# 0xC000005/PyChebyshev

Measured on AMD Instinct MI355X. Metric: point-evals/sec, 5D Black-Scholes n=11^5 barycentric + TT, 1/2/4/8 GPU, higher is better.
Workload: dtype f64; 1 GPU; 5D Black-Scholes n=11^5 full-tensor barycentric, 1,000,000 fp64 queries per GPU; evals_per_point=1, parallelism=batch-sharded x1, model replicated, one process per GPU, gather=none

## Files before the change

include/pcx.h:

```cpp
#ifndef PCX_H
#define PCX_H

#include <stddef.h>
#include <stdint.h>

#ifdef __cplusplus
extern "C" {
#endif

#define PCX_ABI_VERSION 1

#define PCX_OK 0
#define PCX_ERR_INVALID (-1)
#define PCX_ERR_NO_DEVICE (-2)
#define PCX_ERR_HIP (-3)
#define PCX_ERR_UNSUPPORTED (-4)
#define PCX_ERR_NOMEM (-5)

#define PCX_MAX_DIMS 16

typedef struct pcx_bary pcx_bary;
typedef struct pcx_tt pcx_tt;
typedef struct pcx_spline pcx_spline;
typedef struct pcx_slider pcx_slider;
// ... 47 lines not shown
int pcx_bary_derivative_tensor(pcx_bary *h, const int32_t *deriv, double *tensor_out);

int pcx_bary_chebyshev_coefficients(pcx_bary *h, double *coeffs_out);

int pcx_bary_sobol(pcx_bary *h, double *variance_out, double *first_out, double *total_out);

int pcx_tensor_contract_axis(int device, int d, const int32_t *n_nodes, const double *tensor,
                             int axis, const double *vec, double *out);

int pcx_bary_set_kernel(pcx_bary *h, int variant);
int pcx_bary_count_gemms(pcx_bary *h, const int32_t *derivs, int m, int64_t N, int32_t *gemms_out);
int pcx_bary_set_group_tolerance(pcx_bary *h, double tol);
int pcx_bary_set_group_span(pcx_bary *h, int span);
int pcx_bary_kernel_info(pcx_bary *h, int32_t *info_out );
int pcx_bary_grid_info(pcx_bary *h, int32_t *info_out );
int pcx_bary_stream(pcx_bary *h, void **stream);

int pcx_spline_create(int device, int d, const int32_t *n_knots, const double *knots_cat,
                      pcx_bary *const *pieces, int n_pieces, pcx_spline **out);
int pcx_spline_destroy(pcx_spline *h);
int pcx_spline_eval_batch(pcx_spline *h, const double *pts, int64_t N, const int32_t *deriv,
                          double *out);
int pcx_spline_eval_multi_batch(pcx_spline *h, const double *pts, int64_t N, const int32_t *derivs,
                                int m, double *out);
int pcx_spline_piece_ids(pcx_spline *h, const double *pts, int64_t N, int32_t *ids_out);
int pcx_spline_eval_batch_dev(pcx_spline *h, const double *d_pts, int64_t N, const int32_t *deriv,
                              double *d_out);
int pcx_spline_eval_multi_batch_dev(pcx_spline *h, const double *d_pts, int64_t N,
                                    const int32_t *derivs, int m, double *d_out);

// ... 87 lines not shown
```

pychebyshev_amd/_lib.py:

```python
from __future__ import annotations

import ctypes
import os

import numpy as np

HERE = os.path.dirname(os.path.abspath(__file__))
LIB_PATH = os.path.join(HERE, "libpcx_hip.so")

PCX_OK = 0
PCX_ERR_INVALID = -1
PCX_ERR_NO_DEVICE = -2
PCX_ERR_HIP = -3
PCX_ERR_UNSUPPORTED = -4
PCX_ERR_NOMEM = -5


class PcxLibraryError(RuntimeError):
    """libpcx_hip.so is missing, stale, or there is no usable MI355X device."""


class PcxError(RuntimeError):

    def __init__(self, code: int, message: str):
# ... 46 lines not shown
    "pcx_bary_eval_multi_batch_dev": (_I, [_V, _V, _L, c_i32p, _I, _V, _V]),
    "pcx_bary_group_eval_multi_batch": (_I, [c_vpp, _I, c_f64p, _L, c_i32p, _I, c_f64p, _I]),
    "pcx_bary_derivative_tensor": (_I, [_V, c_i32p, c_f64p]),
    "pcx_bary_chebyshev_coefficients": (_I, [_V, c_f64p]),
    "pcx_bary_sobol": (_I, [_V, c_f64p, c_f64p, c_f64p]),
    "pcx_cheb1d_calculus": (_I, [_I, _I, _D, _D, c_f64p, c_f64p, c_f64p, c_f64p, _L, _I, c_f64p, c_i32p, c_f64p, c_f64p]),
    "pcx_bary_calculus_batch": (_I, [_V, _I, c_f64p, c_f64p, c_f64p, _L, _I, c_f64p, c_i32p, c_f64p, c_f64p]),
    "pcx_tt_calculus_batch": (_I, [_V, _I, c_f64p, _L, _I, c_f64p, c_i32p, c_f64p, c_f64p]),
    "pcx_tensor_contract_axis": (_I, [_I, _I, c_i32p, c_f64p, _I, c_f64p, c_f64p]),
    "pcx_bary_set_kernel": (_I, [_V, _I]),
    "pcx_bary_set_group_span": (_I, [_V, _I]),
    "pcx_bary_count_gemms": (_I, [_V, c_i32p, _I, _L, c_i32p]),
    "pcx_bary_set_group_tolerance": (_I, [_V, _D]),
    "pcx_bary_kernel_info": (_I, [_V, c_i32p]),
    "pcx_bary_grid_info": (_I, [_V, c_i32p]),
    "pcx_bary_stream": (_I, [_V, c_vpp]),
    "pcx_spline_create": (_I, [_I, _I, c_i32p, c_f64p, c_vpp, _I, c_vpp]),
    "pcx_spline_destroy": (_I, [_V]),
    "pcx_spline_eval_batch": (_I, [_V, c_f64p, _L, c_i32p, c_f64p]),
    "pcx_spline_eval_multi_batch": (_I, [_V, c_f64p, _L, c_i32p, _I, c_f64p]),
    "pcx_spline_piece_ids": (_I, [_V, c_f64p, _L, c_i32p]),
    "pcx_spline_eval_batch_dev": (_I, [_V, _V, _L, c_i32p, _V]),
    "pcx_spline_eval_multi_batch_dev": (_I, [_V, _V, _L, c_i32p, _I, _V]),
    "pcx_slider_create": (_I, [_I, _I, _I, c_vpp, c_i32p, c_i32p, _D, c_vpp]),
    "pcx_slider_destroy": (_I, [_V]),
    "pcx_slider_eval_batch": (_I, [_V, c_f64p, _L, c_i32p, c_f64p]),
    "pcx_slider_eval_multi_batch": (_I, [_V, c_f64p, _L, c_i32p, _I, c_f64p]),
    "pcx_slider_eval_multi_batch_dev": (_I, [_V, _V, _L, c_i32p, _I, _V]),
    "pcx_tt_create": (_I, [_I, _I, c_i32p, c_i32p, c_f64p, c_f64p, c_f64p, c_i32p, c_vpp]),
    "pcx_tt_destroy": (_I, [_V]),
# ... 139 lines not shown
```

pychebyshev_amd/csrc/bary_kernels.h:

```cpp
#pragma once

#include "pcx_common.h"

static __global__ void k_mode_product(const double *__restrict__ in, double *__restrict__ out,
                               const double *__restrict__ D, long outer, int na, long inner) {
    long idx = (long)blockIdx.x * blockDim.x + threadIdx.x;
    long total = outer * na * inner;
    if (idx >= total) return;
    long q = idx % inner;
    long t = idx / inner;
    int i = (int)(t % na);
    long o = t / na;
    const double *src = in + (o * na) * inner + q;
    const double *drow = D + (long)i * na;
    double s = 0.0;
    for (int j = 0; j < na; ++j) s = __builtin_fma(src[(long)j * inner], drow[j], s);
    out[idx] = s;
}

static __global__ void k_contract_axis(const double *__restrict__ in, double *__restrict__ out,
                                const double *__restrict__ vec, long outer, int na, long inner) {
    long idx = (long)blockIdx.x * blockDim.x + threadIdx.x;
    if (idx >= outer * inner) return;
    long q = idx % inner;
// ... 104 lines not shown
    const uint4 q = reinterpret_cast<const uint4 *>(codes)[4 * t + g];
    return pcx_u4{{q.x, q.y, q.z, q.w}};
}

typedef const pcx_d4 __attribute__((address_space(1))) *pcx_seed_ptr;
template <int R>
struct pcx_seed { pcx_d4 v[R > 0 ? R : 1]; };
template <int R>
__device__ __forceinline__ pcx_seed<R> load_seed(pcx_seed_ptr seed, long t, int g) {
    pcx_seed<R> q;
#pragma unroll
    for (int r = 0; r < R; ++r) q.v[r] = seed[(4 * t + g) * R + r];
    return q;
}

template <int NF>
__device__ __forceinline__ double code_weight_t(unsigned code, const double *bw_col, int PW) {
    if constexpr (NF >= 4) return code_weight(code, bw_col, PW);
    else {
        double w0 = bw_col[(code & 255u) * PW];
        double w1 = bw_col[((code >> 8) & 255u) * PW];
        if constexpr (NF == 3) return (w0 * w1) * bw_col[((code >> 16) & 255u) * PW];
        else return w0 * w1;
    }
}

#define PCX_CHUNK_TILES 4

template <int KS, int NT, bool WIDE, int NF = 4, bool G0 = false, int R = 0>
__global__ void __launch_bounds__(256, 2)
k_bary_mfma(BaryDims dims, BaryMfmaPlan plan, const double *__restrict__ nodes,
            const double *__restrict__ wts, const double *const *__restrict__ frag_tab,
            const unsigned *__restrict__ rowcode, const unsigned *__restrict__ kcode,
            const unsigned *__restrict__ rowcode_hi, const unsigned *__restrict__ kcode_hi,
            const double *__restrict__ pts, double *__restrict__ out, long N, long ostride,
            long ooff, int chunks_per_split, double *__restrict__ partial,
            const int *__restrict__ perm, BaryG0 gs, const double *__restrict__ diff0) {
    static_assert(NT == 1 || NT == 2 || NT == 4, "PW must divide the wave");
    constexpr int PW = 16 * NT;
    constexpr int PH = 64 / PW;
    extern __shared__ double lds[];
    const int lane = threadIdx.x & 63;
    const int wave = threadIdx.x >> 6;
    const int g = lane >> 4;
    const int c = lane & 15;
    double *bw = lds + (size_t)wave * plan.rows * PW;
    const double *bwt = bw + (size_t)plan.tail_base * PW;
    const long base = ((long)blockIdx.x * 4 + wave) * PW;
    typedef const double __attribute__((address_space(1))) *gptr_t;
    const gptr_t frag = (gptr_t)frag_tab[blockIdx.z];
    const pcx_seed_ptr seed = (pcx_seed_ptr)(frag + (size_t)plan.MT * KS * 64);
    const int nchunks = (plan.MT + PCX_CHUNK_TILES - 1) / PCX_CHUNK_TILES;
    const int ch0 = blockIdx.y * chunks_per_split;
    const int ch1 = (ch0 + chunks_per_split < nchunks) ? ch0 + chunks_per_split : nchunks;

    {
        const int pp = lane % PW;
        const int ph = lane / PW;
        const long pidx = base + pp;
        const bool valid = pidx < N;
        const long row = valid ? (perm ? (long)perm[pidx] : pidx) : 0;
        for (int k = ph; k < dims.d; k += PH) {
            const double *nd = nodes + dims.off[k];
            double x = valid ? pts[row * dims.d + k] : nd[0];
            const int trow = dims.off[k] + (k >= plan.split ? 1 : 0);
            bary_weights_1d(x, nd, wts + dims.off[k], dims.n[k], bw + (size_t)trow * PW + pp, PW);
        }
        if (ph == 0) {
            bw[(size_t)(plan.tail_base - 1) * PW + pp] = 1.0;
            bw[(size_t)(plan.rows - 1) * PW + pp] = 1.0;
        }
    }
    __syncthreads();

    double B[NT][KS];
#pragma unroll
    for (int s = 0; s < KS; ++s) {
        unsigned code = kcode[4 * s + g];
#pragma unroll
        for (int nt = 0; nt < NT; ++nt) B[nt][s] = code_weight(code, bwt + 16 * nt + c, PW);
        if (WIDE) {
            unsigned hi = kcode_hi[4 * s + g];
#pragma unroll
            for (int nt = 0; nt < NT; ++nt) B[nt][s] *= code_weight(hi, bwt + 16 * nt + c, PW);
        }
    }
    double ws[NT][R > 0 ? R : 1];
#pragma unroll
    for (int r = 0; r < R; ++r) {
        unsigned code = kcode[4 * KS + r];
#pragma unroll
        for (int nt = 0; nt < NT; ++nt) ws[nt][r] = code_weight(code, bwt + 16 * nt + c, PW);
        if (WIDE) {
            unsigned hi = kcode_hi[4 * KS + r];
#pragma unroll
            for (int nt = 0; nt < NT; ++nt) ws[nt][r] *= code_weight(hi, bwt + 16 * nt + c, PW);
        }
    }

    double total[NT], cs[NT];
#pragma unroll
    for (int nt = 0; nt < NT; ++nt) { total[nt] = 0.0; cs[nt] = 0.0; }
    const gptr_t tf = frag + lane;
    const int t_begin = ch0 * PCX_CHUNK_TILES;
    const int t_end = (ch1 * PCX_CHUNK_TILES < plan.MT) ? ch1 * PCX_CHUNK_TILES : plan.MT;
    const bool split = gridDim.y > 1;
    constexpr bool PIPELINED = (KS >= 12);
    constexpr int DEPTH = 6;
    unsigned cn[4] = {0u, 0u, 0u, 0u}, cnh[4] = {0u, 0u, 0u, 0u};
    double head[DEPTH];
    pcx_d4 acc[NT];
    auto seed_acc = [&](const pcx_seed<R> &sd) {
#pragma unroll
        for (int nt = 0; nt < NT; ++nt) acc[nt] = (pcx_d4){0.0, 0.0, 0.0, 0.0};
#pragma unroll
        for (int r = 0; r < R; ++r)
#pragma unroll
            for (int nt = 0; nt < NT; ++nt)
#pragma unroll
                for (int j = 0; j < 4; ++j) acc[nt][j] = __builtin_fma(sd.v[r][j], ws[nt][r], acc[nt][j]);
    };
    constexpr bool CARRY = PIPELINED && R > 0;
#pragma unroll
    for (int i = 0; i < DEPTH; ++i) head[i] = 0.0;
    if (PIPELINED && t_begin < t_end) {
        if constexpr (R > 0) seed_acc(load_seed<R>(seed, t_begin, g));
        {
            const pcx_u4 q = load_row_codes(rowcode, t_begin, g);
            pcx_u4 qh = q;
            if (WIDE) qh = load_row_codes(rowcode_hi, t_begin, g);
#pragma unroll
            for (int j = 0; j < 4; ++j) {
                cn[j] = q.v[j];
                if (WIDE) cnh[j] = qh.v[j];
            }
        }
#pragma unroll
        for (int i = 0; i < DEPTH; ++i) head[i] = tf[((size_t)t_begin * KS + i) * 64];
    }
    for (int t = t_begin; t < t_end; ++t) {
        double w[NT][4];
        pcx_seed<R> sdn;
        if constexpr (!CARRY) {
            if constexpr (R > 0) sdn = load_seed<R>(seed, t, g);
            seed_acc(sdn);
        }
        const gptr_t tt = tf + (size_t)t * KS * 64;
        if constexpr (PIPELINED) {
            const int t_next = (t + 1 < t_end) ? t + 1 : t;
            const gptr_t tn = tf + (size_t)t_next * KS * 64;
            double ring[DEPTH];
            unsigned cc[4], cch[4];
#pragma unroll
            for (int i = 0; i < DEPTH; ++i) ring[i] = head[i];
            {
                const pcx_u4 q = load_row_codes(rowcode, t_next, g);
                pcx_u4 qh = q;
                if (WIDE) qh = load_row_codes(rowcode_hi, t_next, g);
#pragma unroll
                for (int j = 0; j < 4; ++j) {
                    cc[j] = cn[j];
                    cn[j] = q.v[j];
                    if (WIDE) { cch[j] = cnh[j]; cnh[j] = qh.v[j]; }
                }
            }
            double wr[4][NT][4];
            double wh[4][NT][4];
#pragma unroll
            for (int s = 0; s < KS; ++s) {
                const double a = ring[s % DEPTH];
                if (s + DEPTH < KS) ring[s % DEPTH] = tt[(s + DEPTH) * 64];
                else head[s + DEPTH - KS] = tn[(s + DEPTH - KS) * 64];
                if constexpr (R > 0) {
                    if (s == KS - DEPTH) sdn = load_seed<R>(seed, t_next, g);
                }
#pragma unroll
                for (int j = 0; j < 4; ++j) {
                    if (s == 2 * j) {
#pragma unroll
                        for (int nt = 0; nt < NT; ++nt)
#pragma unroll
                            for (int f = 0; f < (NF < 4 ? NF : 4); ++f)
                                wr[j][nt][f] = bw[(size_t)((cc[j] >> (8 * f)) & 255u) * PW + 16 * nt + c];
                    }
                    if (s == 2 * j + 2) {
#pragma unroll
                        for (int nt = 0; nt < NT; ++nt)
                            w[nt][j] = NF >= 4 ? (wr[j][nt][0] * wr[j][nt][1]) * (wr[j][nt][2] * wr[j][nt][3])
                                     : (NF == 3 ? (wr[j][nt][0] * wr[j][nt][1]) * wr[j][nt][2]
                                                : wr[j][nt][0] * wr[j][nt][1]);
                    }
                    if (WIDE && s == 2 * j + 1) {
#pragma unroll
                        for (int nt = 0; nt < NT; ++nt)
#pragma unroll
                            for (int f = 0; f < 4; ++f)
                                wh[j][nt][f] = bw[(size_t)((cch[j] >> (8 * f)) & 255u) * PW + 16 * nt + c];
                    }
// ... 48 lines not shown
                    v += __shfl_xor(v, 32, 64);
                    if (g == 0) Pl[(size_t)i0 * PW + 16 * nt + c] = v;
                    cs[nt] = 0.0;
                }
            }
            continue;
        }
        const bool chunk_end = ((t + 1) % PCX_CHUNK_TILES == 0) || (t + 1 == plan.MT);
        if (chunk_end) {
            if (split) {
                const int ch = t / PCX_CHUNK_TILES;
#pragma unroll
                for (int nt = 0; nt < NT; ++nt) {
                    long pidx = base + 16 * nt + c;
                    if (pidx < N)
                        partial[(((size_t)blockIdx.z * nchunks + ch) * 4 + g) * (size_t)N + pidx] = cs[nt];
                }
            }
#pragma unroll
            for (int nt = 0; nt < NT; ++nt) { total[nt] += cs[nt]; cs[nt] = 0.0; }
        }
    }

    if constexpr (G0) {
        if (lane < PW) {
            double *Pl = const_cast<double *>(bwt) + lane;
            const long pidx = base + lane;
            const long row = (pidx < N) ? (perm ? (long)perm[pidx] : pidx) : 0;
            bary_g0_finish(gs, diff0, Pl, Pl + (size_t)gs.n0 * PW, bw + (size_t)dims.off[0] * PW + lane, PW,
                           pidx < N ? out + row * ostride + ooff : nullptr);
        }
// ... 161 lines not shown
    }

#pragma unroll
    for (int nt = 0; nt < NT; ++nt) {
        double v = total[nt];
        v += __shfl_xor(v, 16, 64);
        v += __shfl_xor(v, 32, 64);
        long pidx = base + 16 * nt + c;
        if (g == 0 && pidx < N) {
            long row = perm ? (long)perm[pidx] : pidx;
            out[row * ostride + ooff + blockIdx.z] = v;
        }
    }
}

static __global__ void k_bary_reduce(const double *__restrict__ partial, double *__restrict__ out, long N,
                              int nchunks, int nspec, long ostride, long ooff,
                              const int *__restrict__ perm) {
    long idx = (long)blockIdx.x * blockDim.x + threadIdx.x;
    if (idx >= N * nspec) return;
    long p = idx % N;
    int z = (int)(idx / N);
    const double *src = partial + (size_t)z * nchunks * 4 * (size_t)N + p;
    double sg[4];
    for (int g = 0; g < 4; ++g) {
        double t = 0.0;
        for (int ch = 0; ch < nchunks; ++ch) t += src[((size_t)ch * 4 + g) * (size_t)N];
        sg[g] = t;
    }
    long row = perm ? (long)perm[p] : p;
    out[row * ostride + ooff + z] = (sg[0] + sg[1]) + (sg[2] + sg[3]);
}

static __global__ void __launch_bounds__(256)
k_bary_rows(BaryDims dims, int LPP, const double *__restrict__ nodes,
            const double *__restrict__ wts, const double *__restrict__ T,
            const double *__restrict__ pts, double *__restrict__ out, long N, long ostride,
            long ooff, const int *__restrict__ perm) {
    extern __shared__ double lds[];
    const int ppw = 256 / LPP;
    const int pl = threadIdx.x / LPP;
    const int sub = threadIdx.x % LPP;
    const long pidx = (long)blockIdx.x * ppw + pl;
    const bool valid = pidx < N;
    const long row = valid ? (perm ? (long)perm[pidx] : pidx) : 0;
    double *bw = lds + (size_t)pl * dims.sum_n;
// ... 298 lines not shown
```

pychebyshev_amd/csrc/bary_mfma_launch.h:

```cpp
#pragma once

#include "pcx_bary_internal.h"
#include "bary_kernels.h"

static size_t mfma4_lds_bytes(const BaryDims &dm, int ks) {
    return ((size_t)8 * (dm.sum_n + 2) * 32 + (size_t)2 * ks * 64) * sizeof(double);
}

static size_t mfma_lds_bytes(const BaryDims &dm, int nt) {
    return (size_t)4 * (dm.sum_n + 2) * 16 * nt * sizeof(double);
}

template <int KS, int NT, bool WIDE, int NF, int R>
static int launch_mfma_t(pcx_bary *h, const double *const *frag_tab, int m, const double *d_pts, long N,
                         double *d_out, long ostride, long ooff, hipStream_t st, Scratch *split_scratch,
                         const int *perm) {
    const bool allow_split = split_scratch != nullptr;
    size_t lds = mfma_lds_bytes(h->dims, NT);
    auto kern = k_bary_mfma<KS, NT, WIDE, NF, false, R>;
    if (lds > 64 * 1024)
        HIP_TRY(hipFuncSetAttribute((const void *)kern, hipFuncAttributeMaxDynamicSharedMemorySize, (int)lds));
    long per_wg = 4L * 16 * NT;
    long blocks = (N + per_wg - 1) / per_wg;
    if (blocks > 0x7fffffffL) return fail(PCX_ERR_UNSUPPORTED, "batch too large for one launch");
    int nchunks = (h->plan.MT + PCX_CHUNK_TILES - 1) / PCX_CHUNK_TILES;
    int nsplit = 1, cps = nchunks;
    const long want = 512;
    if (allow_split && blocks * m < want && nchunks > 1) {
        nsplit = (int)std::min<long>(nchunks, (want + blocks * m - 1) / (blocks * m));
        cps = (nchunks + nsplit - 1) / nsplit;
        nsplit = (nchunks + cps - 1) / cps;
    }
    double *partial = nullptr;
    if (nsplit > 1) {
        int rc = split_scratch->reserve((size_t)m * nchunks * 4 * (size_t)N * sizeof(double));
        if (rc) return rc;
        partial = (double *)split_scratch->ptr;
    }
    hipLaunchKernelGGL(kern, dim3((unsigned)blocks, (unsigned)nsplit, (unsigned)m), dim3(256), lds, st,
                       h->dims, h->plan, h->d_nodes, h->d_wts, frag_tab, h->d_rowcode, h->d_kcode,
                       h->d_rowcode_hi, h->d_kcode_hi, d_pts, d_out, N, ostride, ooff, cps, partial, perm, BaryG0{}, nullptr);
    HIP_TRY(hipGetLastError());
    if (nsplit > 1) {
        long cnt = N * m;
        hipLaunchKernelGGL(k_bary_reduce, dim3((unsigned)((cnt + 255) / 256)), dim3(256), 0, st, partial, d_out,
                           N, nchunks, m, ostride, ooff, perm);
        HIP_TRY(hipGetLastError());
    }
    return PCX_OK;
}

template <int KS, int R>
static int launch_mfma4_t(pcx_bary *h, const double *const *frag_tab, int m, const double *d_pts, long N,
                          double *d_out, long ostride, long ooff, hipStream_t st, const int *perm) {
    size_t lds = mfma4_lds_bytes(h->dims, KS);
    auto kern = k_bary_mfma4<KS, R>;
    if (lds > 64 * 1024)
        HIP_TRY(hipFuncSetAttribute((const void *)kern, hipFuncAttributeMaxDynamicSharedMemorySize, (int)lds));
    long blocks = (N + 255) / 256;
    if (blocks > 0x7fffffffL) return fail(PCX_ERR_UNSUPPORTED, "batch too large for one launch");
    hipLaunchKernelGGL(kern, dim3((unsigned)blocks, 1, (unsigned)m), dim3(512), lds, st, h->dims, h->plan,
// ... 75 lines not shown

template <int KS, int NF, int R>
static int launch_g0_t(pcx_bary *h, const DerivedTensor &base, const BaryG0 &gs, const double *d_pts, long N, double *d_out,
                       long ostride, long ooff, hipStream_t st) {
    auto kern = k_bary_mfma<KS, 2, false, NF, true, R>;
    const size_t lds = mfma_lds_bytes(h->dims, 2);
    if (lds > 64 * 1024)
        HIP_TRY(hipFuncSetAttribute((const void *)kern, hipFuncAttributeMaxDynamicSharedMemorySize, (int)lds));
    const long blocks = (N + 127) / 128;
    if (blocks > 0x7fffffffL) return fail(PCX_ERR_UNSUPPORTED, "batch too large for one launch");
    BaryMfmaPlan plan = h->plan;
    plan.MT = gs.tps * gs.n0;
    const int nchunks = (plan.MT + PCX_CHUNK_TILES - 1) / PCX_CHUNK_TILES;
    hipLaunchKernelGGL(kern, dim3((unsigned)blocks, 1, 1), dim3(256), lds, st, h->dims, plan, h->d_nodes, h->d_wts,
                       (const double *const *)base.slot_g0, h->d_rowcode_g0, h->d_kcode, nullptr, nullptr, d_pts, d_out, N,
                       ostride, ooff, nchunks, nullptr, nullptr, gs, h->d_diff + h->doff[0]);
    HIP_TRY(hipGetLastError());
    return PCX_OK;
}

template <int NF, int R>
static int launch_g0_nf(pcx_bary *h, const DerivedTensor &base, const BaryG0 &gs, const double *d_pts, long N, double *d_out,
                        long ostride, long ooff, hipStream_t st) {
    switch (h->plan.KS) {
#define CASE_KS(v) case v: return launch_g0_t<v, NF, R>(h, base, gs, d_pts, N, d_out, ostride, ooff, st);
        PCX_CASES_KS_1_32
#undef CASE_KS
    }
    return fail(PCX_ERR_UNSUPPORTED, "no dim-0 group instantiation for KS=%d", h->plan.KS);
}

// ... 22 lines not shown
```

pychebyshev_amd/csrc/pcx_bary.hip:

```cpp

#include "pcx_bary_internal.h"
#include "bary_kernels.h"
#include "bary_mfma_launch.h"
#include "gather_kernels.h"
#include "sobol_kernels.h"

static const int g_g0_span_default = [] { const char *e = getenv("PCX_BARY_G0_SPAN"); return e ? std::min(8, std::max(0, atoi(e))) : 1; }();

static const double g_group_tol_default = [] { const char *e = getenv("PCX_BARY_GROUP_TOL"); double v = e ? atof(e) : 0.0; return v > 0.0 ? v : 3e-13; }();

static const long kSmallTensorElems = 4096;
static const int kCacheSpecs = 96;

static const int kKsList[] = {1, 2, 3, 4, 5, 6, 7, 8, 9, 10, 11, 12, 13, 14, 15, 16, 17, 18, 19, 20, 21, 22,
                              23, 24, 25, 26, 27, 28, 29, 30, 31, 32, 36, 40, 42, 44, 48, 52, 56, 60, 64};

static int pick_ks(int K, int R = 0) {
    int need = (K - R + 3) / 4;
    for (int ks : kKsList)
        if (ks >= need && (ks != 42 || R > 0)) return ks;
    return -1;
}

static int seed_columns(long K, bool seed) {
// ... 31 lines not shown
    PCX_API_BEGIN
    if (!h) return PCX_OK;
    (void)hipSetDevice(h->device);
    if (h->stream) (void)hipStreamSynchronize(h->stream);
    for (auto &kv : h->cache) kv.second.free_all();
    (void)hipFree(h->d_tab);
    h->s_partial.release();
    (void)hipFree(h->d_nodes); (void)hipFree(h->d_wts); (void)hipFree(h->d_diff);
    (void)hipFree(h->d_cheb);
    h->s_cheb[0].release(); h->s_cheb[1].release(); h->s_sobol.release();
    (void)hipFree(h->d_snodes);
    (void)hipFree(h->d_gsnodes);
    (void)hipFree(h->d_rowcode); (void)hipFree(h->d_kcode);
    (void)hipFree(h->d_rowcode_hi); (void)hipFree(h->d_kcode_hi);
    (void)hipFree(h->d_rowcode_g0);
    for (pcx_bary *&r : h->rot) { if (r) pcx_bary_destroy(r); r = nullptr; }
    h->stage.release();
    h->s_rot.release(); h->s_rot2.release();
    if (h->stream) (void)hipStreamDestroy(h->stream);
    delete h;
    return PCX_OK;
    PCX_API_END
}

static int bary_pack(pcx_bary *h, DerivedTensor &dt) {
    if (!h->mfma_ok) return PCX_OK;
    const BaryMfmaPlan &p = h->plan;
    size_t cnt = h->kfold_ok ? bary_kfold_frag_count(h->kf) : (size_t)(h->grid_ok ? h->gp.MT : p.MT) * p.KS * 64;
    const size_t nseed = (size_t)p.MT * 16 * p.R;
    DevBuf frag, slot;
// ... 67 lines not shown
    CREATE_TRY(hipStreamCreateWithFlags(&h->stream, hipStreamNonBlocking));
    CREATE_TRY(hipMalloc((void **)&h->d_nodes, sum_n * sizeof(double)));
    CREATE_TRY(hipMalloc((void **)&h->d_wts, sum_n * sizeof(double)));
    CREATE_TRY(hipMalloc((void **)&h->d_diff, sum_n2 * sizeof(double)));
    CREATE_TRY(hipMemcpy(h->d_nodes, nodes_cat, sum_n * sizeof(double), hipMemcpyHostToDevice));
    CREATE_TRY(hipMemcpy(h->d_wts, weights_cat, sum_n * sizeof(double), hipMemcpyHostToDevice));
    CREATE_TRY(hipMemcpy(h->d_diff, diffmat_cat, sum_n2 * sizeof(double), hipMemcpyHostToDevice));

    long Mrows = total / h->dims.n[d - 1];
    int lpp = 1;
    while (lpp < 64 && lpp < Mrows) lpp <<= 1;
    while (lpp < 64 && (size_t)(256 / lpp) * sum_n * sizeof(double) > 48 * 1024) lpp <<= 1;
    h->lpp = lpp;

    { const char *e = getenv("PCX_BARY_SEED"); h->seed = !(e && e[0] == '0'); }
    h->mfma_ok = plan_mfma(h->dims, h->plan, h->seed);
    if (h->mfma_ok) {
        const bool narrow = h->plan.split <= PCX_CODE_FIELDS && d - h->plan.split <= PCX_CODE_FIELDS;
        h->nt = (h->plan.KS <= 32 || (narrow && h->plan.KS <= 40)) ? 2 : 1;
        if (mfma_lds_bytes(h->dims, h->nt) > 150 * 1024) h->nt = 1;
        if (mfma_lds_bytes(h->dims, h->nt) > 150 * 1024) h->mfma_ok = false;
    }
    if (!h->mfma_ok && (size_t)(256 / h->lpp) * sum_n * sizeof(double) > 160 * 1024) {
        int c_ = fail(PCX_ERR_UNSUPPORTED, "sum of node counts %ld too large for any kernel (MFMA plan: each of the "
                      "head / tail parts <= %d rows and a tail product <= 256; row kernel: sum <= 5120)", sum_n, PCX_MAX_PART_ROWS);
        pcx_bary_destroy(h);
        return c_;
    }
    h->mfma4_ok = h->mfma_ok && mfma4_lds_bytes(h->dims, h->plan.KS) <= 160 * 1024 &&
                  h->plan.KS <= 32 && h->plan.split <= PCX_CODE_FIELDS && d - h->plan.split <= PCX_CODE_FIELDS;
// ... 47 lines not shown
        auto lane_order = [&](std::vector<unsigned> &v) {
            std::vector<unsigned> o(v.size());
            for (long t = 0; t < (long)p.MT; ++t)
                for (int g = 0; g < 4; ++g)
                    for (int j = 0; j < 4; ++j) o[(size_t)(4 * t + g) * 4 + j] = v[(size_t)16 * t + g + 4 * j];
            v.swap(o);
        };
        lane_order(rowcode);
        lane_order(rowcode_hi);
        if (h->wide) {
            CREATE_TRY(hipMalloc((void **)&h->d_rowcode_hi, rowcode_hi.size() * sizeof(unsigned)));
            CREATE_TRY(hipMemcpy(h->d_rowcode_hi, rowcode_hi.data(), rowcode_hi.size() * sizeof(unsigned), hipMemcpyHostToDevice));
        }
        CREATE_TRY(hipMalloc((void **)&h->d_rowcode, rowcode.size() * sizeof(unsigned)));
        CREATE_TRY(hipMemcpy(h->d_rowcode, rowcode.data(), rowcode.size() * sizeof(unsigned), hipMemcpyHostToDevice));
        long M1 = 1;
        for (int k = 1; k < p.split; ++k) M1 *= h->dims.n[k];
        if (!h->wide && p.split >= 2 && p.split <= PCX_CODE_FIELDS && h->nt == 2 && p.KS <= 32 && M1 >= 16 &&
            2 * h->dims.n[0] <= p.rows - p.tail_base && h->dims.n[0] >= 2 && h->dims.n[0] <= 16) {
            const int tps = (int)((M1 + 15) / 16);
            const long mtg = (long)tps * h->dims.n[0];
            if (mtg * 100 <= (long)p.MT * 115) {
                std::vector<unsigned> rc((size_t)mtg * 16);
                for (long t = 0; t < mtg; ++t)
                    for (int r = 0; r < 16; ++r) {
                        const long m1 = (t % tps) * 16 + r;
                        unsigned f[PCX_CODE_FIELDS] = {ones_h, ones_h, ones_h, ones_h};
                        if (m1 < M1) {
                            long rem = m1;
                            for (int k = p.split - 1; k >= 1; --k) {
// ... 1151 lines not shown
extern "C" int pcx_bary_kernel_info(pcx_bary *h, int32_t *info) {
    PCX_API_BEGIN
    if (!h || !info) return fail(PCX_ERR_INVALID, "NULL argument");
    { const int keep = h->variant; h->variant = 0; info[0] = bary_effective_variant(h); h->variant = keep; }
    info[1] = h->mfma_ok ? (h->kfold_ok ? h->kf.MT : (h->grid_ok ? h->gp.MT : h->plan.MT)) : 0;
    info[2] = h->mfma_ok ? (h->kfold_ok ? h->kf.nbody * h->kf.P : h->plan.KS) : 0;
    info[3] = h->mfma_ok ? (int32_t)(h->kfold_ok ? bary_kfold_lds_bytes(h->kf, h->nt)
                                                  : (h->grid_ok ? bary_grid_lds_bytes(h, h->nt) : mfma_lds_bytes(h->dims, h->nt)))
                         : (256 / h->lpp) * h->dims.sum_n * 8;
    info[4] = h->mfma_ok ? 64 * h->nt : 256 / h->lpp;
    info[5] = h->mfma_ok ? h->plan.split : h->dims.d - 1;
    return PCX_OK;
    PCX_API_END
}

extern "C" int pcx_bary_grid_info(pcx_bary *h, int32_t *info) {
    PCX_API_BEGIN
    if (!h || !info) return fail(PCX_ERR_INVALID, "NULL argument");
    info[0] = h->grid_ok ? 1 : (h->kfold_ok ? 2 : 0);
    info[1] = h->grid_ok ? h->gp.RA : 0;
    info[2] = h->grid_ok ? h->gp.MT : (h->kfold_ok ? h->kf.MT : 0);
    info[3] = h->grid_ok ? h->gp.nchunks : (h->kfold_ok ? h->kf.KS2 : 0);
    return PCX_OK;
    PCX_API_END
}

extern "C" int pcx_bary_stream(pcx_bary *h, void **stream) {
    PCX_API_BEGIN
    if (!h || !stream) return fail(PCX_ERR_INVALID, "NULL argument");
    *stream = (void *)h->stream;
// ... 4 lines not shown
```

pychebyshev_amd/csrc/pcx_bary_internal.h:

```cpp
#pragma once

#include "pcx_internal.h"

static int alloc_plain(DevBuf &b, long total) {
    int rc = b.alloc(((size_t)total + PCX_PLAIN_PAD) * sizeof(double));
    if (rc) return rc;
    HIP_TRY(hipMemset((char *)b.p + (size_t)total * sizeof(double), 0, PCX_PLAIN_PAD * sizeof(double)));
    return PCX_OK;
}

struct DerivedTensor {
    double *plain = nullptr;
    double *frag = nullptr;
    double **slot = nullptr;
    double *frag_g0 = nullptr;
    double **slot_g0 = nullptr;
    uint64_t last_use = 0;
    void free_all() {
        if (plain) (void)hipFree(plain);
        if (frag) (void)hipFree(frag);
        if (slot) (void)hipFree(slot);
        if (frag_g0) (void)hipFree(frag_g0);
        if (slot_g0) (void)hipFree(slot_g0);
        plain = frag = frag_g0 = nullptr;
// ... 6 lines not shown
    hipStream_t stream = nullptr;
    BaryDims dims;
    long total = 0;
    std::vector<int> doff;
    double *d_nodes = nullptr, *d_wts = nullptr, *d_diff = nullptr;
    double *d_cheb = nullptr;
    Scratch s_cheb[2];
    Scratch s_sobol;
    bool mfma_ok = false;
    bool seed = true;
    BaryMfmaPlan plan;
    int nt = 2;
    unsigned *d_rowcode = nullptr, *d_kcode = nullptr;
    unsigned *d_rowcode_hi = nullptr, *d_kcode_hi = nullptr;
    bool wide = false;
    bool grid_ok = false;
    BaryGridPlan gp;
    double *d_gsnodes = nullptr;
    bool kfold_ok = false;
    BaryKfoldPlan kf;
    bool grid_prod = false;
    bool g0_ok = false;
    int g0_tps = 0;
    int g0_nf = 2;
    unsigned *d_rowcode_g0 = nullptr;
    int g0_span = 1;
    pcx_bary *rot[PCX_MAX_DIMS] = {};
    char rot_state[PCX_MAX_DIMS] = {};
    Scratch s_rot, s_rot2;
    std::map<std::vector<int>, double> pair_dev;
// ... 77 lines not shown
```

pychebyshev_amd/csrc/pcx_common.h:

```cpp
#pragma once

#include <hip/hip_runtime.h>
#include <stdint.h>

#include "../../include/pcx.h"

#define PCX_WAVE 64

typedef double pcx_d4 __attribute__((ext_vector_type(4)));

#define PCX_MAX_PART_ROWS 255
#define PCX_CODE_FIELDS 4

struct BaryDims {
    int d;
    int sum_n;
    int n[PCX_MAX_DIMS];
    int off[PCX_MAX_DIMS];
};

struct BaryMfmaPlan {
    int split;
    int M;
    int K;
// ... 32 lines not shown
    int str;
    int P;
    int nbody;
};

#define PCX_G0_MAX 9
struct BaryG0 {
    int nmem;
    int maxorder;
    int tps;
    int n0;
    int order[PCX_G0_MAX];
    int col[PCX_G0_MAX];
};

#define PCX_PLAIN_PAD 64

struct BarySmallScale {
    double s[4];
};

struct SplinePieceModel {
    const double *snodes, *nodes, *wts;
    const double *T;
    const double *const *T_tab;
    BarySmallScale sc;
};

struct TTDims {
    int d;
// ... 8 lines not shown
```

Baseline: 206.3 million point-evals/s.

## Split tail wave of MFMA bary blocks across chunks and precompute row byte offsets

The tail blocks left after the last full wave of resident workgroups are split across tile chunks, with a partial-sum reduction afterwards, so the final wave keeps more CUs busy. The split target now comes from an occupancy query instead of a fixed constant. The pipelined loop reads precomputed LDS byte offsets in place of 8-bit row codes and loads the next tile's codes partway through the current tile. The tail-weight setup uses a two-field variant when few dimensions remain, and the reduction kernel is rewritten with one wave per chunk group and unrolled loads. The cost is extra partial-buffer traffic and a reduce launch for tail blocks, plus more device memory for the offset tables.

```diff
diff --git a/include/pcx.h b/include/pcx.h
--- a/include/pcx.h
+++ b/include/pcx.h
@@ -85,6 +85,7 @@
 int pcx_bary_set_group_span(pcx_bary *h, int span);
 int pcx_bary_kernel_info(pcx_bary *h, int32_t *info_out );
 int pcx_bary_grid_info(pcx_bary *h, int32_t *info_out );
+int pcx_bary_tail_info(pcx_bary *h, int32_t *info_out );
 int pcx_bary_stream(pcx_bary *h, void **stream);
 
 int pcx_spline_create(int device, int d, const int32_t *n_knots, const double *knots_cat,
diff --git a/pychebyshev_amd/_lib.py b/pychebyshev_amd/_lib.py
--- a/pychebyshev_amd/_lib.py
+++ b/pychebyshev_amd/_lib.py
@@ -84,6 +84,7 @@
     "pcx_bary_set_group_tolerance": (_I, [_V, _D]),
     "pcx_bary_kernel_info": (_I, [_V, c_i32p]),
     "pcx_bary_grid_info": (_I, [_V, c_i32p]),
+    "pcx_bary_tail_info": (_I, [_V, c_i32p]),
     "pcx_bary_stream": (_I, [_V, c_vpp]),
     "pcx_spline_create": (_I, [_I, _I, c_i32p, c_f64p, c_vpp, _I, c_vpp]),
     "pcx_spline_destroy": (_I, [_V]),
diff --git a/pychebyshev_amd/csrc/bary_kernels.h b/pychebyshev_amd/csrc/bary_kernels.h
--- a/pychebyshev_amd/csrc/bary_kernels.h
+++ b/pychebyshev_amd/csrc/bary_kernels.h
@@ -1,4 +1,6 @@
 #pragma once
+
+#include <type_traits>
 
 #include "pcx_common.h"
 
@@ -142,6 +144,11 @@
     return q;
 }
 
+__device__ __forceinline__ pcx_u4 load_row_offs(const unsigned *__restrict__ offs, long t, int g, int w) {
+    const uint4 q = reinterpret_cast<const uint4 *>(offs)[8 * t + 2 * g + w];
+    return pcx_u4{{q.x, q.y, q.z, q.w}};
+}
+
 template <int NF>
 __device__ __forceinline__ double code_weight_t(unsigned code, const double *bw_col, int PW) {
     if constexpr (NF >= 4) return code_weight(code, bw_col, PW);
@@ -163,7 +170,8 @@
             const unsigned *__restrict__ rowcode_hi, const unsigned *__restrict__ kcode_hi,
             const double *__restrict__ pts, double *__restrict__ out, long N, long ostride,
             long ooff, int chunks_per_split, double *__restrict__ partial,
-            const int *__restrict__ perm, BaryG0 gs, const double *__restrict__ diff0) {
+            const int *__restrict__ perm, BaryG0 gs, const double *__restrict__ diff0,
+            const unsigned *__restrict__ rowoff, BaryTail tail) {
     static_assert(NT == 1 || NT == 2 || NT == 4, "PW must divide the wave");
     constexpr int PW = 16 * NT;
     constexpr int PH = 64 / PW;
@@ -174,13 +182,27 @@
     const int c = lane & 15;
     double *bw = lds + (size_t)wave * plan.rows * PW;
     const double *bwt = bw + (size_t)plan.tail_base * PW;
-    const long base = ((long)blockIdx.x * 4 + wave) * PW;
+    int bx = blockIdx.x;
+    const int nchunks = (plan.MT + PCX_CHUNK_TILES - 1) / PCX_CHUNK_TILES;
+    int ch0 = blockIdx.y * chunks_per_split, ch_len = chunks_per_split;
+    bool split = gridDim.y > 1;
+    long part_p0 = 0;
+    long part_n = N;
+    if (!G0 && tail.P > 0 && bx >= tail.first) {
+        const int e = bx - tail.first;
+        const int tb = e / tail.P;
+        bx = tail.first + tb;
+        ch0 = (e - tb * tail.P) * tail.cpp;
+        ch_len = tail.cpp;
+        split = true;
+        part_p0 = (long)tail.first * 4 * PW;
+        part_n = N - part_p0;
+    }
+    const int ch1 = (ch0 + ch_len < nchunks) ? ch0 + ch_len : nchunks;
+    const long base = ((long)bx * 4 + wave) * PW;
     typedef const double __attribute__((address_space(1))) *gptr_t;
     const gptr_t frag = (gptr_t)frag_tab[blockIdx.z];
     const pcx_seed_ptr seed = (pcx_seed_ptr)(frag + (size_t)plan.MT * KS * 64);
-    const int nchunks = (plan.MT + PCX_CHUNK_TILES - 1) / PCX_CHUNK_TILES;
-    const int ch0 = blockIdx.y * chunks_per_split;
-    const int ch1 = (ch0 + chunks_per_split < nchunks) ? ch0 + chunks_per_split : nchunks;
 
     {
         const int pp = lane % PW;
@@ -202,29 +224,34 @@
     __syncthreads();
 
     double B[NT][KS];
-#pragma unroll
-    for (int s = 0; s < KS; ++s) {
-        unsigned code = kcode[4 * s + g];
-#pragma unroll
-        for (int nt = 0; nt < NT; ++nt) B[nt][s] = code_weight(code, bwt + 16 * nt + c, PW);
-        if (WIDE) {
-            unsigned hi = kcode_hi[4 * s + g];
-#pragma unroll
-            for (int nt = 0; nt < NT; ++nt) B[nt][s] *= code_weight(hi, bwt + 16 * nt + c, PW);
-        }
-    }
     double ws[NT][R > 0 ? R : 1];
-#pragma unroll
-    for (int r = 0; r < R; ++r) {
-        unsigned code = kcode[4 * KS + r];
-#pragma unroll
-        for (int nt = 0; nt < NT; ++nt) ws[nt][r] = code_weight(code, bwt + 16 * nt + c, PW);
-        if (WIDE) {
-            unsigned hi = kcode_hi[4 * KS + r];
-#pragma unroll
-            for (int nt = 0; nt < NT; ++nt) ws[nt][r] *= code_weight(hi, bwt + 16 * nt + c, PW);
-        }
-    }
+    auto tail_weights = [&](auto nft) {
+        constexpr int NFT = decltype(nft)::value;
+#pragma unroll
+        for (int s = 0; s < KS; ++s) {
+            unsigned code = kcode[4 * s + g];
+#pragma unroll
+            for (int nt = 0; nt < NT; ++nt) B[nt][s] = code_weight_t<NFT>(code, bwt + 16 * nt + c, PW);
+            if (WIDE) {
+                unsigned hi = kcode_hi[4 * s + g];
+#pragma unroll
+                for (int nt = 0; nt < NT; ++nt) B[nt][s] *= code_weight(hi, bwt + 16 * nt + c, PW);
+            }
+        }
+#pragma unroll
+        for (int r = 0; r < R; ++r) {
+            unsigned code = kcode[4 * KS + r];
+#pragma unroll
+            for (int nt = 0; nt < NT; ++nt) ws[nt][r] = code_weight_t<NFT>(code, bwt + 16 * nt + c, PW);
+            if (WIDE) {
+                unsigned hi = kcode_hi[4 * KS + r];
+#pragma unroll
+                for (int nt = 0; nt < NT; ++nt) ws[nt][r] *= code_weight(hi, bwt + 16 * nt + c, PW);
+            }
+        }
+    };
+    if (!WIDE && dims.d - plan.split <= 2) tail_weights(std::integral_constant<int, 2>{});
+    else tail_weights(std::integral_constant<int, 4>{});
 
     double total[NT], cs[NT];
 #pragma unroll
@@ -232,10 +259,32 @@
     const gptr_t tf = frag + lane;
     const int t_begin = ch0 * PCX_CHUNK_TILES;
     const int t_end = (ch1 * PCX_CHUNK_TILES < plan.MT) ? ch1 * PCX_CHUNK_TILES : plan.MT;
-    const bool split = gridDim.y > 1;
     constexpr bool PIPELINED = (KS >= 12);
     constexpr int DEPTH = 6;
-    unsigned cn[4] = {0u, 0u, 0u, 0u}, cnh[4] = {0u, 0u, 0u, 0u};
+    constexpr bool OFFS = PIPELINED && !WIDE && !G0;
+    constexpr bool CODE2 = WIDE || (OFFS && NF >= 3);
+    constexpr int CODE_STEP = 8;
+    unsigned cc[4] = {0u, 0u, 0u, 0u}, cch[4] = {0u, 0u, 0u, 0u};
+    auto load_codes = [&](long t) {
+        const pcx_u4 q = OFFS ? load_row_offs(rowoff, t, g, 0) : load_row_codes(rowcode, t, g);
+        pcx_u4 qh = q;
+        if constexpr (WIDE) qh = load_row_codes(rowcode_hi, t, g);
+        else if constexpr (CODE2) qh = load_row_offs(rowoff, t, g, 1);
+#pragma unroll
+        for (int j = 0; j < 4; ++j) {
+            cc[j] = q.v[j];
+            if (CODE2) cch[j] = qh.v[j];
+        }
+    };
+    auto head_entry = [&](int j, int nt, int f) -> double {
+        if constexpr (OFFS) {
+            const unsigned word = f < 2 ? cc[j] : cch[j];
+            const unsigned off = (f & 1) ? (word >> 16) : (word & 0xffffu);
+            return *reinterpret_cast<const double *>(reinterpret_cast<const char *>(bw + 16 * nt + c) + off);
+        } else {
+            return bw[(size_t)((cc[j] >> (8 * f)) & 255u) * PW + 16 * nt + c];
+        }
+    };
     double head[DEPTH];
     pcx_d4 acc[NT];
     auto seed_acc = [&](const pcx_seed<R> &sd) {
@@ -253,16 +302,7 @@
     for (int i = 0; i < DEPTH; ++i) head[i] = 0.0;
     if (PIPELINED && t_begin < t_end) {
         if constexpr (R > 0) seed_acc(load_seed<R>(seed, t_begin, g));
-        {
-            const pcx_u4 q = load_row_codes(rowcode, t_begin, g);
-            pcx_u4 qh = q;
-            if (WIDE) qh = load_row_codes(rowcode_hi, t_begin, g);
-#pragma unroll
-            for (int j = 0; j < 4; ++j) {
-                cn[j] = q.v[j];
-                if (WIDE) cnh[j] = qh.v[j];
-            }
-        }
+        load_codes(t_begin);
 #pragma unroll
         for (int i = 0; i < DEPTH; ++i) head[i] = tf[((size_t)t_begin * KS + i) * 64];
     }
@@ -278,20 +318,8 @@
             const int t_next = (t + 1 < t_end) ? t + 1 : t;
             const gptr_t tn = tf + (size_t)t_next * KS * 64;
             double ring[DEPTH];
-            unsigned cc[4], cch[4];
 #pragma unroll
             for (int i = 0; i < DEPTH; ++i) ring[i] = head[i];
-            {
-                const pcx_u4 q = load_row_codes(rowcode, t_next, g);
-                pcx_u4 qh = q;
-                if (WIDE) qh = load_row_codes(rowcode_hi, t_next, g);
-#pragma unroll
-                for (int j = 0; j < 4; ++j) {
-                    cc[j] = cn[j];
-                    cn[j] = q.v[j];
-                    if (WIDE) { cch[j] = cnh[j]; cnh[j] = qh.v[j]; }
-                }
-            }
             double wr[4][NT][4];
             double wh[4][NT][4];
 #pragma unroll
@@ -302,6 +330,7 @@
                 if constexpr (R > 0) {
                     if (s == KS - DEPTH) sdn = load_seed<R>(seed, t_next, g);
                 }
+                if (s == CODE_STEP) load_codes(t_next);
 #pragma unroll
                 for (int j = 0; j < 4; ++j) {
                     if (s == 2 * j) {
@@ -309,7 +338,7 @@
                         for (int nt = 0; nt < NT; ++nt)
 #pragma unroll
                             for (int f = 0; f < (NF < 4 ? NF : 4); ++f)
-                                wr[j][nt][f] = bw[(size_t)((cc[j] >> (8 * f)) & 255u) * PW + 16 * nt + c];
+                                wr[j][nt][f] = head_entry(j, nt, f);
                     }
                     if (s == 2 * j + 2) {
 #pragma unroll
@@ -388,7 +417,7 @@
                 for (int nt = 0; nt < NT; ++nt) {
                     long pidx = base + 16 * nt + c;
                     if (pidx < N)
-                        partial[(((size_t)blockIdx.z * nchunks + ch) * 4 + g) * (size_t)N + pidx] = cs[nt];
+                        partial[(((size_t)blockIdx.z * nchunks + ch) * 4 + g) * (size_t)part_n + (pidx - part_p0)] = cs[nt];
                 }
             }
 #pragma unroll
@@ -580,22 +609,34 @@
     }
 }
 
-static __global__ void k_bary_reduce(const double *__restrict__ partial, double *__restrict__ out, long N,
-                              int nchunks, int nspec, long ostride, long ooff,
-                              const int *__restrict__ perm) {
-    long idx = (long)blockIdx.x * blockDim.x + threadIdx.x;
-    if (idx >= N * nspec) return;
-    long p = idx % N;
-    int z = (int)(idx / N);
-    const double *src = partial + (size_t)z * nchunks * 4 * (size_t)N + p;
-    double sg[4];
-    for (int g = 0; g < 4; ++g) {
-        double t = 0.0;
-        for (int ch = 0; ch < nchunks; ++ch) t += src[((size_t)ch * 4 + g) * (size_t)N];
-        sg[g] = t;
-    }
-    long row = perm ? (long)perm[p] : p;
-    out[row * ostride + ooff + z] = (sg[0] + sg[1]) + (sg[2] + sg[3]);
+static __global__ void __launch_bounds__(256)
+k_bary_reduce(const double *__restrict__ partial, double *__restrict__ out, long N, int nchunks, int nspec,
+              long ostride, long ooff, const int *__restrict__ perm, long p0) {
+    __shared__ double sg[4][64];
+    const int lane = threadIdx.x & 63;
+    const int g = threadIdx.x >> 6;
+    const long idx = (long)blockIdx.x * 64 + lane;
+    const bool valid = idx < N * nspec;
+    const long p = valid ? idx % N : 0;
+    const int z = valid ? (int)(idx / N) : 0;
+    const double *src = partial + ((size_t)z * nchunks * 4 + g) * (size_t)N + p;
+    const size_t step = (size_t)4 * (size_t)N;
+    double t = 0.0;
+    int ch = 0;
+    for (; ch + 8 <= nchunks; ch += 8) {
+        double v[8];
+#pragma unroll
+        for (int i = 0; i < 8; ++i) v[i] = src[(size_t)(ch + i) * step];
+#pragma unroll
+        for (int i = 0; i < 8; ++i) t += v[i];
+    }
+    for (; ch < nchunks; ++ch) t += src[(size_t)ch * step];
+    sg[g][lane] = t;
+    __syncthreads();
+    if (g == 0 && valid) {
+        long row = perm ? (long)perm[p0 + p] : p0 + p;
+        out[row * ostride + ooff + z] = (sg[0][lane] + sg[1][lane]) + (sg[2][lane] + sg[3][lane]);
+    }
 }
 
 static __global__ void __launch_bounds__(256)
diff --git a/pychebyshev_amd/csrc/bary_mfma_launch.h b/pychebyshev_amd/csrc/bary_mfma_launch.h
--- a/pychebyshev_amd/csrc/bary_mfma_launch.h
+++ b/pychebyshev_amd/csrc/bary_mfma_launch.h
@@ -11,6 +11,15 @@
     return (size_t)4 * (dm.sum_n + 2) * 16 * nt * sizeof(double);
 }
 
+static int resident_slots(const void *kern, size_t lds, int device, int *slots) {
+    int per_cu = 0, cus = 0;
+    HIP_TRY(hipOccupancyMaxActiveBlocksPerMultiprocessor(&per_cu, kern, 256, lds));
+    HIP_TRY(hipDeviceGetAttribute(&cus, hipDeviceAttributeMultiprocessorCount, device));
+    *slots = (int)std::max<long>(1, std::min<long>(512, (long)per_cu * cus));
+    return PCX_OK;
+}
+
+static const long kTailMinWork = 2048;
 template <int KS, int NT, bool WIDE, int NF, int R>
 static int launch_mfma_t(pcx_bary *h, const double *const *frag_tab, int m, const double *d_pts, long N,
                          double *d_out, long ostride, long ooff, hipStream_t st, Scratch *split_scratch,
@@ -25,26 +34,51 @@
     if (blocks > 0x7fffffffL) return fail(PCX_ERR_UNSUPPORTED, "batch too large for one launch");
     int nchunks = (h->plan.MT + PCX_CHUNK_TILES - 1) / PCX_CHUNK_TILES;
     int nsplit = 1, cps = nchunks;
-    const long want = 512;
+    if (KS >= 12 && !WIDE && !h->d_rowoff[NT - 1]) return fail(PCX_ERR_UNSUPPORTED, "row offsets of the pipelined loop were not built");
+    if (!h->slots[NT - 1]) {
+        int rc = resident_slots((const void *)kern, lds, h->device, &h->slots[NT - 1]);
+        if (rc) return rc;
+    }
+    if (h->slots_query) return PCX_OK;
+    const long want = h->slots[NT - 1];
     if (allow_split && blocks * m < want && nchunks > 1) {
         nsplit = (int)std::min<long>(nchunks, (want + blocks * m - 1) / (blocks * m));
         cps = (nchunks + nsplit - 1) / nsplit;
         nsplit = (nchunks + cps - 1) / cps;
     }
+    BaryTail tail{0, 0, 0};
+    long grid_x = blocks;
+    const long tail_blocks = blocks % want;
+    const bool tail_pays = h->tail_mode == 2 || (h->tail_mode == 1 && (long)h->plan.MT * (KS + 5) * NT >= kTailMinWork);
+    if (tail_pays && allow_split && m == 1 && nsplit == 1 && nchunks > 1 && blocks > want && tail_blocks > 0 &&
+        2 * tail_blocks <= want) {
+        int P = (int)std::min<long>(nchunks, want / tail_blocks);
+        tail.cpp = (nchunks + P - 1) / P;
+        P = (nchunks + tail.cpp - 1) / tail.cpp;
+        if (P > 1 && blocks + want <= 0x7fffffffL) {
+            tail.first = (int)(blocks - tail_blocks);
+            tail.P = P;
+            grid_x = tail.first + tail_blocks * P;
+        }
+    }
+    h->last_tail_P = tail.P;
+    h->last_tail_blocks = tail.P ? (int)tail_blocks : 0;
+    const long part_p0 = tail.P ? (long)tail.first * per_wg : 0;
     double *partial = nullptr;
-    if (nsplit > 1) {
-        int rc = split_scratch->reserve((size_t)m * nchunks * 4 * (size_t)N * sizeof(double));
+    if (nsplit > 1 || tail.P) {
+        int rc = split_scratch->reserve((size_t)m * nchunks * 4 * (size_t)(N - part_p0) * sizeof(double));
         if (rc) return rc;
         partial = (double *)split_scratch->ptr;
     }
-    hipLaunchKernelGGL(kern, dim3((unsigned)blocks, (unsigned)nsplit, (unsigned)m), dim3(256), lds, st,
+    hipLaunchKernelGGL(kern, dim3((unsigned)grid_x, (unsigned)nsplit, (unsigned)m), dim3(256), lds, st,
                        h->dims, h->plan, h->d_nodes, h->d_wts, frag_tab, h->d_rowcode, h->d_kcode,
-                       h->d_rowcode_hi, h->d_kcode_hi, d_pts, d_out, N, ostride, ooff, cps, partial, perm, BaryG0{}, nullptr);
+                       h->d_rowcode_hi, h->d_kcode_hi, d_pts, d_out, N, ostride, ooff, cps, partial, perm, BaryG0{}, nullptr,
+                       h->d_rowoff[NT - 1], tail);
     HIP_TRY(hipGetLastError());
-    if (nsplit > 1) {
-        long cnt = N * m;
-        hipLaunchKernelGGL(k_bary_reduce, dim3((unsigned)((cnt + 255) / 256)), dim3(256), 0, st, partial, d_out,
-                           N, nchunks, m, ostride, ooff, perm);
+    if (nsplit > 1 || tail.P) {
+        long cnt = (N - part_p0) * m;
+        hipLaunchKernelGGL(k_bary_reduce, dim3((unsigned)((cnt + 63) / 64)), dim3(256), 0, st, partial, d_out,
+                           N - part_p0, nchunks, m, ostride, ooff, perm, part_p0);
         HIP_TRY(hipGetLastError());
     }
     return PCX_OK;
@@ -150,7 +184,7 @@
     const int nchunks = (plan.MT + PCX_CHUNK_TILES - 1) / PCX_CHUNK_TILES;
     hipLaunchKernelGGL(kern, dim3((unsigned)blocks, 1, 1), dim3(256), lds, st, h->dims, plan, h->d_nodes, h->d_wts,
                        (const double *const *)base.slot_g0, h->d_rowcode_g0, h->d_kcode, nullptr, nullptr, d_pts, d_out, N,
-                       ostride, ooff, nchunks, nullptr, nullptr, gs, h->d_diff + h->doff[0]);
+                       ostride, ooff, nchunks, nullptr, nullptr, gs, h->d_diff + h->doff[0], nullptr, BaryTail{0, 0, 0});
     HIP_TRY(hipGetLastError());
     return PCX_OK;
 }
diff --git a/pychebyshev_amd/csrc/pcx_bary.hip b/pychebyshev_amd/csrc/pcx_bary.hip
--- a/pychebyshev_amd/csrc/pcx_bary.hip
+++ b/pychebyshev_amd/csrc/pcx_bary.hip
@@ -69,6 +69,7 @@
     (void)hipFree(h->d_rowcode); (void)hipFree(h->d_kcode);
     (void)hipFree(h->d_rowcode_hi); (void)hipFree(h->d_kcode_hi);
     (void)hipFree(h->d_rowcode_g0);
+    (void)hipFree(h->d_rowoff[0]); (void)hipFree(h->d_rowoff[1]);
     for (pcx_bary *&r : h->rot) { if (r) pcx_bary_destroy(r); r = nullptr; }
     h->stage.release();
     h->s_rot.release(); h->s_rot2.release();
@@ -166,6 +167,7 @@
     h->lpp = lpp;
 
     { const char *e = getenv("PCX_BARY_SEED"); h->seed = !(e && e[0] == '0'); }
+    { const char *e = getenv("PCX_BARY_TAIL"); h->tail_mode = (e && e[0] == '0') ? 0 : ((e && e[0] == '2') ? 2 : 1); }
     h->mfma_ok = plan_mfma(h->dims, h->plan, h->seed);
     if (h->mfma_ok) {
         const bool narrow = h->plan.split <= PCX_CODE_FIELDS && d - h->plan.split <= PCX_CODE_FIELDS;
@@ -243,6 +245,20 @@
         }
         CREATE_TRY(hipMalloc((void **)&h->d_rowcode, rowcode.size() * sizeof(unsigned)));
         CREATE_TRY(hipMemcpy(h->d_rowcode, rowcode.data(), rowcode.size() * sizeof(unsigned), hipMemcpyHostToDevice));
+        if (!h->wide && p.KS >= 12) {
+            std::vector<unsigned> offs((size_t)p.MT * 32);
+            for (int nt = 1; nt <= 2; ++nt) {
+                const unsigned sc = 16u * nt * sizeof(double);
+                for (size_t q = 0; q < (size_t)p.MT * 4; ++q)
+                    for (int j = 0; j < 4; ++j) {
+                        const unsigned code = rowcode[4 * q + j];
+                        offs[8 * q + j] = ((code & 255u) * sc) | ((((code >> 8) & 255u) * sc) << 16);
+                        offs[8 * q + 4 + j] = (((code >> 16) & 255u) * sc) | (((code >> 24) * sc) << 16);
+                    }
+                CREATE_TRY(hipMalloc((void **)&h->d_rowoff[nt - 1], offs.size() * sizeof(unsigned)));
+                CREATE_TRY(hipMemcpy(h->d_rowoff[nt - 1], offs.data(), offs.size() * sizeof(unsigned), hipMemcpyHostToDevice));
+            }
+        }
         long M1 = 1;
         for (int k = 1; k < p.split; ++k) M1 *= h->dims.n[k];
         if (!h->wide && p.split >= 2 && p.split <= PCX_CODE_FIELDS && h->nt == 2 && p.KS <= 32 && M1 >= 16 &&
@@ -1424,6 +1440,34 @@
     PCX_API_END
 }
 
+extern "C" int pcx_bary_tail_info(pcx_bary *h, int32_t *info) {
+    PCX_API_BEGIN
+    if (!h || !info) return fail(PCX_ERR_INVALID, "NULL argument");
+    for (int i = 0; i < 6; ++i) info[i] = 0;
+    std::lock_guard<std::mutex> lk(h->mu);
+    if (!h->mfma_ok || h->kfold_ok || h->grid_ok) return PCX_OK;
+    if (!h->slots[h->nt - 1]) {
+        int rc = use_device(h->device);
+        if (rc) return rc;
+        h->slots_query = true;
+        switch (h->plan.R) {
+        case 1: rc = bary_launch_rowcode_seed1(h, nullptr, 1, nullptr, 65536, nullptr, 1, 0, h->stream, nullptr, nullptr); break;
+        case 2: rc = bary_launch_rowcode_seed2(h, nullptr, 1, nullptr, 65536, nullptr, 1, 0, h->stream, nullptr, nullptr); break;
+        default: rc = launch_rowcode<0>(h, nullptr, 1, nullptr, 65536, nullptr, 1, 0, h->stream, nullptr, nullptr);
+        }
+        h->slots_query = false;
+        if (rc) return rc;
+    }
+    info[0] = h->slots[h->nt - 1];
+    info[1] = 64 * h->nt;
+    info[2] = (h->plan.MT + PCX_CHUNK_TILES - 1) / PCX_CHUNK_TILES;
+    info[3] = h->tail_mode;
+    info[4] = h->last_tail_P;
+    info[5] = h->last_tail_blocks;
+    return PCX_OK;
+    PCX_API_END
+}
+
 extern "C" int pcx_bary_grid_info(pcx_bary *h, int32_t *info) {
     PCX_API_BEGIN
     if (!h || !info) return fail(PCX_ERR_INVALID, "NULL argument");
diff --git a/pychebyshev_amd/csrc/pcx_bary_internal.h b/pychebyshev_amd/csrc/pcx_bary_internal.h
--- a/pychebyshev_amd/csrc/pcx_bary_internal.h
+++ b/pychebyshev_amd/csrc/pcx_bary_internal.h
@@ -44,6 +44,11 @@
     unsigned *d_rowcode = nullptr, *d_kcode = nullptr;
     unsigned *d_rowcode_hi = nullptr, *d_kcode_hi = nullptr;
     bool wide = false;
+    unsigned *d_rowoff[2] = {nullptr, nullptr};
+    int tail_mode = 1;
+    int slots[2] = {0, 0};
+    int last_tail_P = 0, last_tail_blocks = 0;
+    bool slots_query = false;
     bool grid_ok = false;
     BaryGridPlan gp;
     double *d_gsnodes = nullptr;
diff --git a/pychebyshev_amd/csrc/pcx_common.h b/pychebyshev_amd/csrc/pcx_common.h
--- a/pychebyshev_amd/csrc/pcx_common.h
+++ b/pychebyshev_amd/csrc/pcx_common.h
@@ -70,6 +70,12 @@
     int col[PCX_G0_MAX];
 };
 
+struct BaryTail {
+    int first;
+    int P;
+    int cpp;
+};
+
 #define PCX_PLAIN_PAD 64
 
 struct BarySmallScale {
```

Measured after the change: 211.4 million point-evals/s, median of 6. 2.5% higher.
